# aconz2/font-ocr

Hardware: AMD Instinct MI355X
Metric: Mpixels/s scanned (95-glyph x --x-bits=2 bank) (higher is better)
Workload: dtype i8

## Files before the change

### font_ocr_amd/csrc/hip/common.h

```cpp
#pragma once

#include <hip/hip_runtime.h>

#include <algorithm>
#include <cstddef>
#include <cstdint>
#include <cstdio>
#include <mutex>
#include <string>
#include <vector>

#include "devmem.h"
#include "focr_ncc.h"

namespace focr_dec {
struct VerifyRec;
}

namespace focr {

struct VerifyMeta;

struct SizeClass {
    uint32_t n_w, n_h;
// ... 99 lines not shown
    uint32_t row_max = 0;
    uint32_t seg_shift = 0;
    void reset() { *this = SizeEstimate{}; }
    double margin() const { return std::min(0.2, std::max(0.04, 3.0 * var)); }
    uint64_t row_bound() const { return (uint64_t)row_max + row_max / 4 + 16; }
    void update(const focr_ctx *c, uint64_t n_cand, uint64_t n_hits, uint64_t largest_row);
    void adopt(uint64_t sig);
    void publish(uint64_t sig) const;
    static void forget(uint64_t sig);
};

}

constexpr uint32_t COUNTER_WORDS = 64, QUEUE_XCDS = 8, QUEUE_STRIDE = 32, MAX_SCAN_QUEUES = 128;
constexpr uint32_t TAIL_DONE_WORD = 56, ORDER_DONE_WORD = 57;
constexpr uint32_t LIVE_WORD0 = 8, LIVE_WORDS = 40;
static_assert(LIVE_WORD0 + LIVE_WORDS <= TAIL_DONE_WORD && ORDER_DONE_WORD < COUNTER_WORDS, "d_counter's named words overlap");
constexpr size_t COUNTER_BYTES = (COUNTER_WORDS + (size_t)MAX_SCAN_QUEUES * QUEUE_XCDS * QUEUE_STRIDE) * sizeof(uint32_t);

struct ResultBlock {
    uint64_t candidates;
    uint64_t hits;
    uint64_t matches;
    uint64_t lines_chars;
    uint64_t flags;
    uint64_t row_max;
    uint64_t tail_hits;
    uint64_t host_hits;
};
enum ResSlot : uint32_t { RES_CANDIDATES, RES_HITS, RES_MATCHES, RES_LINES_CHARS, RES_FLAGS, RES_ROW_MAX, RES_TAIL_HITS, RES_HOST_HITS, RES_SLOTS };
static_assert(sizeof(ResultBlock) == 64 && sizeof(ResultBlock) == RES_SLOTS * sizeof(uint64_t), "the result block is eight words");
static_assert(offsetof(ResultBlock, candidates) == 8 * RES_CANDIDATES && offsetof(ResultBlock, hits) == 8 * RES_HITS && offsetof(ResultBlock, matches) == 8 * RES_MATCHES &&
// ... 212 lines not shown
                     unsigned long long capacity, int rust);
int reserve_hits(focr_ctx *c, size_t want);
int launch_scan_mfma(focr_ctx *ctx, float threshold);
int launch_clear(focr_ctx *c, const focr::ClearList &l);
int pass_stats(focr_ctx *c, const ScanPlan &P, size_t si, double thr_d);
bool pass_appends(const focr_ctx *c, const SuperClass &su);
int build_mfma_bank(focr_ctx *ctx, const uint8_t *needles);
void layout_supers(focr_ctx *c);
int quantise_bank(focr_ctx *c, const uint8_t *dense, std::vector<int8_t> &qbank, std::vector<uint32_t> &tglobal, std::vector<uint32_t> &order_of);
bool rows_applicable(const focr_ctx *c);
uint32_t rows_capacity_for(uint64_t row_max);
void row_segments(const focr_ctx *c, uint32_t *seg_shift, uint32_t *n_seg);
size_t row_buckets(const focr_ctx *c);
unsigned tail_grid(const focr_ctx *c, unsigned blocks);
int rows2_begin(focr_ctx *c, ClearList &clear);
int rows2_place(focr_ctx *c, const unsigned long long *n_cand_p, size_t ub_c, size_t ub_h, bool big_expected, bool sort);
int rows2_verify(focr_ctx *c, double thr_d, const unsigned long long *n_cand_p, size_t ub_c);
int legacy_verify(focr_ctx *c, double thr_d, const unsigned long long *n_cand_p, size_t ub_c, float *sims, uint64_t *flags);
int sort_keys_u64(focr_ctx *c, DevArray<uint64_t> &keys, DevArray<uint64_t> &keys_alt, size_t n, unsigned end_bit);
int sort_pairs_u64_f32(focr_ctx *c, DevArray<uint64_t> &keys, DevArray<uint64_t> &keys_alt, DevArray<float> &vals, DevArray<float> &vals_alt, size_t n, unsigned end_bit);
int exclusive_scan_u64(focr_ctx *c, const uint64_t *in, uint64_t *out, size_t n);
int compact_candidates(focr_ctx *c, const uint64_t *keys, const float *sims, const uint64_t *flags, uint64_t *pos,
                       const unsigned long long *n_cand_p, size_t ub_c);
int order_sorted_hits(focr_ctx *c, uint64_t *hkeys, float *hsims, const uint64_t *n_p, size_t ub, const unsigned long long *n_cand_p, size_t ub_c);
int order_hits(focr_ctx *ctx);
int materialise_matches(focr_ctx *c, hipStream_t s);
void bank_host_prepare(focr_ctx *c, const focr_template_t *templates, size_t n_templates, const uint8_t *needles,
                       std::vector<uint32_t> &direct, std::vector<uint8_t> &dense);
void ctx_share_stream(focr_ctx *c, hipStream_t lane_stream, hipStream_t io_stream);
int wait_batch(focr_ctx *c);
int pages_alt_ingest(focr_ctx *c, const void *d_luma, size_t n_pages, size_t r_w, size_t r_h, int invert, hipStream_t s);
int pages_alt_swap(focr_ctx *c, size_t n_pages, size_t r_w, size_t r_h);
// ... 35 lines not shown
```

### font_ocr_amd/csrc/hip/ctx.hip

```cpp
#include <algorithm>
#include <cmath>
#include <cstring>
#include <mutex>

#include "common.h"

namespace focr {

static std::mutex g_err_mu;
static std::string g_err;

void set_global_error(const std::string &s) {
    std::lock_guard<std::mutex> lk(g_err_mu);
    g_err = s;
}

int fail(focr_ctx *ctx, int code, const std::string &msg) {
    if (ctx) ctx->err = msg;
    set_global_error(msg);
    return code;
}

static void free_bank(focr_ctx *c) {
    c->bank = {};
// ... 141 lines not shown

int focr_debug_set_tail_grid(focr_ctx_t *c, uint32_t num, uint32_t den) {
    if (!c) return FOCR_ERR_INVALID;
    c->dbg_grid_num = num;
    c->dbg_grid_den = den;
    return FOCR_OK;
}

int focr_debug_set_stats_form(focr_ctx_t *c, int form) {
    if (!c || form < 0 || form > 1) return FOCR_ERR_INVALID;
    c->dbg_stats_form = form;
    return FOCR_OK;
}

int focr_debug_set_verify_form(focr_ctx_t *c, int form) {
    if (!c || form < 0 || form > 1) return FOCR_ERR_INVALID;
    c->dbg_verify_form = form;
    return FOCR_OK;
}

int focr_sync(focr_ctx_t *c) {
    if (!c) return FOCR_ERR_INVALID;
    FOCR_HIP(c, hipSetDevice(c->device));
    if (c->sizes_pending || c->post_pending) return finish_results(c);
    return wait_batch(c);
}

int focr_bank_upload(focr_ctx_t *c, const focr_template_t *templates, size_t n_templates, const uint8_t *needles,
                     size_t needles_len) {
    if (!c || !templates || !n_templates || !needles) return fail(c, FOCR_ERR_INVALID, "focr_bank_upload: bad arguments");
    if (n_templates > 65535) return fail(c, FOCR_ERR_INVALID, "focr_bank_upload: more than 65535 templates");
// ... 145 lines not shown
```

### font_ocr_amd/csrc/hip/rows.hip

```cpp
#include "common.h"

namespace focr {

constexpr uint32_t XBINS = 1024;
template <int CAP, int WAVES, bool LIST, bool PAY>
__global__ __launch_bounds__(WAVES * 64) void row_sort_kernel(uint32_t n_rows, const uint32_t *__restrict__ base, const uint32_t *__restrict__ fill,
                                                              uint64_t *__restrict__ bucket, uint32_t sub_bits, uint32_t bt, uint32_t seg_mask, uint32_t xs, uint32_t n_bins,
                                                              uint32_t *__restrict__ big, unsigned long long *__restrict__ flags_word, float *__restrict__ pay,
                                                              unsigned long long limit) {
    extern __shared__ __attribute__((aligned(16))) uint32_t sort_lds[];
    constexpr int K = CAP / 64;
    const int lane = threadIdx.x & 63, wv = threadIdx.x >> 6;
    uint32_t *cur = sort_lds + (size_t)wv * (XBINS + 1 + CAP);
    uint32_t *out = cur + XBINS + 1;
    const uint32_t wave = __builtin_amdgcn_readfirstlane(blockIdx.x * WAVES + wv), n_waves = gridDim.x * WAVES;
    const uint64_t sub_mask = (1ull << sub_bits) - 1;
    const uint32_t n_items = LIST ? min(big[0], n_rows) : n_rows;
    uint32_t it = wave, r = 0, n = 0, b = 0;
    if (it < n_items) {
        r = LIST ? big[1 + it] : it;
        n = fill[r];
        b = base[r];
    }
    while (it < n_items) {
// ... 73 lines not shown
#pragma unroll
            for (int k = 0; k < K; k++)
                if (64u * k < n && (uint32_t)lane + 64u * k < n) {
                    const uint32_t e = sub[k], bin = ((e >> bt) & seg_mask) >> xs, lo = cur[bin], hi = cur[bin + 1];
                    uint32_t rank = 0;
                    for (uint32_t i = lo; i < hi; i++) rank += out[i] < e;
                    row[lo + rank] = high | e;
                    if (PAY) pay[b + lo + rank] = pv[k];
                }
            __builtin_amdgcn_fence(__ATOMIC_ACQ_REL, "wavefront");
        }
        it = it2, r = r2, n = n2, b = b2;
    }
}

__global__ __launch_bounds__(256) void hit_scatter_kernel(const uint64_t *__restrict__ cand, const unsigned long long *__restrict__ n_cand_p, unsigned long long cap,
                                                          const RowHist rows, const uint32_t *__restrict__ hbase, const float *__restrict__ sims,
                                                          const uint32_t *__restrict__ slots, uint64_t *__restrict__ hkeys, float *__restrict__ hsims,
                                                          unsigned long long hit_cap) {
    const unsigned long long n = min(*n_cand_p, cap);
    const unsigned long long stride = (unsigned long long)gridDim.x * blockDim.x;
    for (unsigned long long i = (unsigned long long)blockIdx.x * blockDim.x + threadIdx.x; i < n; i += stride) {
        const uint32_t slot = slots[i];
        if (slot == 0xffffffffu) continue;
        const uint64_t key = cand[i];
        const unsigned long long pos = (unsigned long long)hbase[row_of_key(key, rows)] + slot;
        if (pos < hit_cap) {
            hkeys[pos] = key;
            hsims[pos] = sims[i];
        }
    }
}


void row_segments(const focr_ctx *c, uint32_t *seg_shift, uint32_t *n_seg) {
    uint32_t sh = c->est.seg_shift;
    if (!sh) {
        while (((size_t)1 << sh) < c->pages.r_w) sh++;
        while (sh > 5 && ((size_t)1 << sh) * c->n_templates > ((size_t)1 << 19)) sh--;
    }
    *seg_shift = sh;
    *n_seg = (uint32_t)((c->pages.r_w + ((size_t)1 << sh) - 1) >> sh);
}

// ... 20 lines not shown
    if (!clear.add(big, 8)) return fail(c, FOCR_ERR_INVALID, "rows: clear list full or region too large");
    uint32_t seg_shift, n_seg;
    row_segments(c, &seg_shift, &n_seg);
    c->row_hist = RowHist{nullptr, (uint32_t)c->pages.r_h, c->fmt.bt + c->fmt.bx, c->fmt.by, (uint32_t)c->sub_p0, c->fmt.bt, c->fmt.bx, seg_shift, n_seg};
    return FOCR_OK;
}

uint32_t rows_capacity_for(uint64_t row_max) { return row_max <= 4096 ? 4096u : 0u; }

unsigned tail_grid(const focr_ctx *c, unsigned blocks) {
    if (!c->dbg_grid_num || !c->dbg_grid_den) return blocks;
    return (unsigned)std::max<uint64_t>(1, (uint64_t)blocks * c->dbg_grid_num / c->dbg_grid_den);
}


int rows2_place(focr_ctx *c, const unsigned long long *n_cand_p, size_t ub_c, size_t ub_h, bool big_expected, bool sort) {
    const uint32_t n_rows = (uint32_t)row_buckets(c);
    int rc;
    if ((rc = reserve_hits(c, ub_h + 1))) return rc;
    const unsigned cus = c->n_cus;
    const uint32_t *hits = (const uint32_t *)c->rows_hits.p, *hbase = (const uint32_t *)c->rows_hbase.p;
    if (ub_c) {
        const unsigned nb = tail_grid(c, (unsigned)std::max<size_t>(1, std::min<size_t>((ub_c + 255) / 256, (size_t)cus * 16)));
        hipLaunchKernelGGL(hit_scatter_kernel, dim3(nb), dim3(256), 0, c->stream, (const uint64_t *)c->d_cand, n_cand_p, (unsigned long long)ub_c, c->row_hist, hbase,
                           (const float *)c->scan_pos.p, (const uint32_t *)c->scan_flags.p, c->d_hit_keys, c->d_hit_sims_alt, (unsigned long long)c->d_hit_keys.cap);
        FOCR_HIP(c, hipGetLastError());
    }
    if (!sort) return FOCR_OK;
    unsigned long long *flags_word = (unsigned long long *)&c->d_res.p->flags;
    const unsigned row_blocks = tail_grid(c, (unsigned)std::max<size_t>(1, std::min<size_t>(((size_t)n_rows + 3) / 4, (size_t)cus * 8)));
    const uint32_t seg_w = 1u << c->row_hist.seg_shift;
    uint32_t xs = 0;
    while ((seg_w >> xs) > XBINS) xs++;
    const uint32_t n_bins = seg_w >> xs;
    uint32_t *big = (uint32_t *)c->rows_big.p;
    auto k1 = row_sort_kernel<1024, 4, false, true>;
    auto k2 = row_sort_kernel<4096, 1, true, true>;
    const size_t lds1 = (size_t)4 * (XBINS + 1 + 1024) * 4, lds2 = (size_t)(XBINS + 1 + 4096) * 4;
    hipLaunchKernelGGL(k1, dim3(row_blocks), dim3(256), lds1, c->stream, n_rows, hbase, hits, c->d_hit_keys, c->fmt.bt + c->fmt.bx, c->fmt.bt, seg_w - 1, xs, n_bins,
                       big_expected ? big : (uint32_t *)nullptr, flags_word, c->d_hit_sims_alt, (unsigned long long)c->d_hit_keys.cap);
// ... 11 lines not shown
```

### font_ocr_amd/csrc/hip/scan_mfma.hip

```cpp
#include <algorithm>
#include <cmath>
#include <mutex>

#include "mfma_common.h"

namespace focr {

struct TurnChain {
    std::mutex mu;
    static constexpr unsigned RING = 8;
    hipEvent_t ev[RING] = {};
    unsigned n = 0;
};
static TurnChain scan_turns[64], stats_turns[64];

struct Turn {
    focr_ctx *c;
    TurnChain &chain;
    std::lock_guard<std::mutex> lock;
    bool entered = false;
    Turn(focr_ctx *c, TurnChain &chain) : c(c), chain(chain), lock(chain.mu) {}
    int begin() {
        for (hipEvent_t &e : chain.ev)
            if (!e) FOCR_HIP(c, hipEventCreateWithFlags(&e, hipEventDisableTiming));
// ... 145 lines not shown
                }
                if (rc) return rc;
                t0 = t1;
            }
        }
    }
    for (size_t k = 0; k < c->bank.classes.size(); k++) {
        const SizeClass &sc = c->bank.classes[k];
        if (!sc.tall || sc.n_w >= c->pages.r_w || sc.n_h >= c->pages.r_h) continue;
        if ((rc = launch_scan_tall(c, k, thr_d, c->d_cand, nullptr, c->d_counter.as<unsigned long long>() + 1, (unsigned long long)c->ub_cand, 0))) return rc;
    }
    return FOCR_OK;
}

static int row_tail(focr_ctx *c, double thr_d, const unsigned long long *n_cand_p, size_t ub_c) {
    int rc = rows2_verify(c, thr_d, n_cand_p, ub_c);
    if (rc) return rc;
    size_t ub_h = std::min(ub_c, c->est.hits);
    uint64_t row_max = c->est.row_bound();
    if (!c->estimated) {
        uint64_t hits = 0;
        FOCR_HIP(c, hipMemcpyAsync(&hits, &c->d_res.p->tail_hits, sizeof(uint64_t), hipMemcpyDeviceToHost, c->stream));
        FOCR_HIP(c, hipMemcpyAsync(&row_max, &c->d_res.p->row_max, sizeof(uint64_t), hipMemcpyDeviceToHost, c->stream));
        FOCR_HIP(c, hipStreamSynchronize(c->stream));
        ub_h = (size_t)hits;
    }
    c->row_cap = rows_capacity_for(row_max);
    const bool big_expected = row_max > 1024, sort_rows = c->row_cap != 0;
    c->tail_path.big_launch = sort_rows && big_expected;
    c->tail_path.library_sort = !sort_rows && ub_h >= 2;
    c->tail_path.seg_shift = c->row_hist.seg_shift;
    c->tail_path.n_seg = c->row_hist.n_seg;
    if ((rc = rows2_place(c, n_cand_p, ub_c, ub_h, big_expected, sort_rows))) return rc;
    if (!sort_rows && (rc = sort_pairs_u64_f32(c, c->d_hit_keys, c->d_hit_keys_alt, c->d_hit_sims_alt, c->d_hit_sims, ub_h, c->fmt.bits()))) return rc;
    return order_sorted_hits(c, c->d_hit_keys, c->d_hit_sims_alt, &c->d_res.p->tail_hits, ub_h, n_cand_p, ub_c);
}

static int legacy_tail(focr_ctx *c, double thr_d, const unsigned long long *n_cand_p, size_t ub_c) {
    c->row_cap = 0;
    int rc = reserve_hits(c, ub_c + 1);
    if (rc) return rc;
    if (!c->scratch(c->scan_flags, (ub_c + 1) * 8) || !c->scratch(c->scan_pos, (ub_c + 1) * 8)) return fail(c, FOCR_ERR_NOMEM, "scan_mfma: hipMalloc failed");
    uint64_t *flags = c->scan_flags.as<uint64_t>(), *pos = c->scan_pos.as<uint64_t>();
    if (c->d_cand_alt.reserve(c->d_cand.cap, Grow::exact, &c->stream)) return fail(c, FOCR_ERR_NOMEM, "scan_mfma: hipMalloc(cand_alt) failed");
    if ((rc = sort_keys_u64(c, c->d_cand, c->d_cand_alt, ub_c, c->fmt.bits()))) return rc;
    if ((rc = legacy_verify(c, thr_d, n_cand_p, ub_c, c->d_hit_sims, flags))) return rc;
    FOCR_HIP(c, hipEventRecord(c->ev[EV_VERIFY_END], c->stream));
    if ((rc = compact_candidates(c, c->d_cand, c->d_hit_sims, flags, pos, n_cand_p, ub_c))) return rc;
// ... 64 lines not shown
```

### font_ocr_amd/csrc/hip/verify.h

```cpp
#pragma once
#include "common.h"

namespace focr {

typedef int v4i __attribute__((ext_vector_type(4)));
typedef v4i v4i_b1 __attribute__((aligned(1)));
typedef int v3i __attribute__((ext_vector_type(3)));
typedef v3i v3i_b1 __attribute__((aligned(1)));
typedef unsigned int v2u __attribute__((ext_vector_type(2)));

struct VerifyMeta {
    double s_n, n_recip, rnorm_n;
    uint16_t n_w, n_h;
    uint32_t row0;
};
static_assert(sizeof(VerifyMeta) == 32, "VerifyMeta is staged in LDS as two 16-byte words per template (verify_plan.h: VERIFY_RECORD_BYTES)");
struct VerifyArgs {
    const uint8_t *pages;
    uint32_t pitch, rows_alloc;
    KeyFmt fmt;
    const uint32_t *order_of;
    const TemplateConst *tc;
    const v4i *needles16;
    const uint32_t *needle16_row;
// ... 35 lines not shown
    const uint32_t r = emit ? row_of_key(key, rows) : 0xffffffffu;
    uint32_t slot = 0xffffffffu;
    uint64_t todo = __builtin_amdgcn_ballot_w64(emit);
    while (todo) {
        const uint32_t r0 = (uint32_t)__builtin_amdgcn_readlane((int)r, (int)__builtin_ctzll(todo));
        const uint64_t peers = __builtin_amdgcn_ballot_w64(r == r0);
        uint32_t start = 0;
        if (lane == (int)__builtin_ctzll(peers)) start = atomicAdd(row_hits + r0, (uint32_t)__builtin_popcountll(peers));
        start = (uint32_t)__builtin_amdgcn_readlane((int)start, (int)__builtin_ctzll(peers));
        if (r == r0) slot = start + __builtin_amdgcn_mbcnt_hi((uint32_t)(peers >> 32), __builtin_amdgcn_mbcnt_lo((uint32_t)peers, 0u));
        todo &= ~peers;
    }
    return slot;
}


__device__ __forceinline__ bool verify_candidate(uint64_t key, const VerifyArgs &va, float *sim_out) {
    const VerifyFrame f = verify_frame(key, va);
    if (f.bad) return verify_reject(va, sim_out);
    const uint32_t ci = va.order_of[f.t];
    const TemplateConst c = va.tc[ci];
    const uint32_t halves = c.n_w > 16 ? 2 : 1;
    const uint32_t row0 = va.needle16_row[ci];
    const v4i *nd = va.needles16 + row0;
    const uint8_t *pg = f.window(va);
    uint32_t acc = 0, s_p = 0, s2_p = 0;
    for (uint32_t hf = 0; hf < halves; hf++) {
        const uint32_t w_here = min(c.n_w - 16 * hf, 16u);
        v4i keep;
#pragma unroll
// ... 137 lines not shown
```

### font_ocr_amd/csrc/hip/verify.hip

```cpp
#include "tail_block.h"
#include "verify.h"
#include "verify_plan.h"

namespace focr {

static VerifyArgs verify_args(const focr_ctx *c, double thr_d) {
    return VerifyArgs{c->pages.u8, (uint32_t)c->pages.pitch, (uint32_t)c->pages.rows_alloc, c->fmt, c->bank.d_order_of, c->bank.d_tconst,
                      c->bank.d_needles16.as<const v4i>(), c->bank.d_needle16_row, thr_d, c->bank.d_vmeta.p,
                      (uint32_t)c->n_templates, (uint32_t)c->n_pages,
                      (uint32_t)c->pages.r_w, (uint32_t)c->pages.r_h, (unsigned long long *)&c->d_res.p->flags};
}

__global__ __launch_bounds__(1024) void row_prefix_kernel(const uint32_t *__restrict__ cnt, uint32_t n, uint32_t *__restrict__ base,
                                                          uint32_t *__restrict__ zero, uint64_t *__restrict__ total_out,
                                                          uint64_t *__restrict__ max_out) {
    __shared__ uint32_t wave_sum[16], wave_max[16];
    row_prefix_block(cnt, n, base, zero, total_out, max_out, wave_sum, wave_max);
}

template <int MODE>
__global__ __launch_bounds__(VERIFY_THREADS, MODE >= 2 ? 8 : 1) void verify_list_kernel(
    const uint64_t *__restrict__ cand, const unsigned long long *__restrict__ n_cand_p, unsigned long long cap, const VerifyArgs va, uint32_t lds_rows, uint32_t n_h,
    const RowHist rows, float *__restrict__ sims, uint32_t *__restrict__ slots, uint32_t *__restrict__ row_hits, const TailWork tw) {
    extern __shared__ __attribute__((aligned(16))) v4i verify_lds[];
    __shared__ uint32_t wave_sum[16], wave_max[16];
    constexpr bool LDS = MODE == 1;
    VerifyMeta *meta = reinterpret_cast<VerifyMeta *>(verify_lds);
    v4i *needle_lds = verify_lds + 2 * va.n_templates;
    uint32_t *needle12 = reinterpret_cast<uint32_t *>(needle_lds);
    v2u *needle8 = reinterpret_cast<v2u *>(needle_lds + va.n_templates);
    for (uint32_t i = threadIdx.x; i < 2 * va.n_templates; i += blockDim.x) verify_lds[i] = reinterpret_cast<const v4i *>(va.vmeta)[i];
    if (MODE == 1)
        for (uint32_t i = threadIdx.x; i < lds_rows; i += blockDim.x) needle_lds[i] = va.needles16[i];
    if (MODE == 2)
        for (uint32_t i = threadIdx.x; i < lds_rows; i += blockDim.x) {
            const v4i r = va.needles16[i];
            needle12[3 * i] = (uint32_t)r[0], needle12[3 * i + 1] = (uint32_t)r[1], needle12[3 * i + 2] = (uint32_t)r[2];
        }
// ... 5 lines not shown
        for (uint32_t i = threadIdx.x; i < 4 * va.n_templates; i += blockDim.x) {
            const uint32_t t = i >> 2, q = i & 3, row0 = va.vmeta[t].row0;
            uint32_t d = 0;
#pragma unroll
            for (uint32_t k = 0; k < 4; k++)
                if (4 * q + k < n_h) d |= ((uint32_t)va.needles16[row0 + 4 * q + k][2] & 0xffu) << (8 * k);
            reinterpret_cast<uint32_t *>(needle_lds)[i] = d;
        }
    }
    __syncthreads();
    const unsigned long long n = min(*n_cand_p, cap);
    const int lane = threadIdx.x & 63;
    const unsigned long long stride = (unsigned long long)gridDim.x * blockDim.x;
    const unsigned long long first = (unsigned long long)blockIdx.x * blockDim.x + (threadIdx.x & ~63u);
    uint64_t key_next = first + lane < n ? cand[first + lane] : 0;
    for (unsigned long long i0 = first; i0 < n; i0 += stride) {
        const unsigned long long i = i0 + lane;
        const bool valid = i < n;
        const uint64_t key = key_next;
        if (i + stride < n) key_next = cand[i + stride];
        float sim = 0.f;
        const bool emit = valid && (MODE == 3   ? verify_candidate_w89(key, va, needle8, needle_lds, meta, &sim)
                                    : MODE == 2 ? verify_candidate_narrow(key, va, needle12, meta, &sim)
                                                : verify_candidate_meta<LDS>(key, va, needle_lds, meta, &sim));
        const uint32_t slot = claim_slot(emit, key, rows, row_hits, lane);
        if (valid) {
            sims[i] = sim;
            slots[i] = slot;
        }
    }
    if (last_workgroup(tw.done)) row_prefix_block(row_hits, tw.n_rows, tw.hbase, nullptr, tw.total_out, tw.max_out, wave_sum, wave_max);
}

template <int ROWB>
__global__ __launch_bounds__(VERIFY_THREADS, 4) void verify_chunks_kernel(
    const uint64_t *__restrict__ cand, const unsigned long long *__restrict__ n_cand_p, unsigned long long cap, const VerifyArgs va, const ChunkTable ct,
    const uint32_t *__restrict__ vrows_t, const VerifyMeta *__restrict__ vmeta_t, const RowHist rows, float *__restrict__ sims, uint32_t *__restrict__ slots,
    uint32_t *__restrict__ row_hits, const TailWork tw) {
    extern __shared__ __attribute__((aligned(16))) v4i verify_lds[];
    __shared__ uint32_t wave_sum[16], wave_max[16];
    constexpr uint32_t ROWDW = ROWB / 4;
    VerifyMeta *meta = reinterpret_cast<VerifyMeta *>(verify_lds);
    const int lane = threadIdx.x & 63, wv = threadIdx.x >> 6;
    uint64_t *q_base = reinterpret_cast<uint64_t *>(verify_lds + ct.data_bytes / 16);
    uint64_t *q_key = q_base + (size_t)wv * CHUNK_QUEUE;
    uint32_t *q_pos = reinterpret_cast<uint32_t *>(q_base + (size_t)(VERIFY_THREADS / 64) * CHUNK_QUEUE) + (size_t)wv * CHUNK_QUEUE;
    const unsigned long long n = min(*n_cand_p, cap);
    const unsigned long long n_waves = (unsigned long long)gridDim.x * (VERIFY_THREADS / 64);
    const unsigned long long per_wave = ((n + n_waves - 1) / n_waves + 63) / 64 * 64;
    const unsigned long long wb = min(n, ((unsigned long long)blockIdx.x * (VERIFY_THREADS / 64) + wv) * per_wave), we = min(n, wb + per_wave);
    auto step = [&](uint32_t m, const VerifyMeta *meta_c, const uint32_t *rows_c) {
        const bool valid = (uint32_t)lane < m;
        const uint64_t key = valid ? q_key[lane] : 0;
        const uint32_t pos = valid ? q_pos[lane] : 0;
        float sim = 0.f;
        bool emit = false;
        if (valid) {
            if (ROWB == 12) emit = verify_candidate_narrow(key, va, rows_c, meta_c, &sim);
            else emit = verify_candidate_meta<true>(key, va, reinterpret_cast<const v4i *>(rows_c), meta_c, &sim);
        }
        const uint32_t slot = claim_slot(emit, key, rows, row_hits, lane);
        if (valid && pos < n) {
            sims[pos] = sim;
            slots[pos] = slot;
        }
    };
    for (uint32_t k = 0; k < ct.n; k++) {
        const uint32_t t_lo = ct.t_lo[k], t_hi = ct.t_lo[k + 1], row_lo = ct.row_lo[k], n_rows_c = ct.row_lo[k + 1] - row_lo;
        uint32_t *rows_lds = reinterpret_cast<uint32_t *>(verify_lds + 2 * (t_hi - t_lo));
        __syncthreads();
        for (uint32_t i = threadIdx.x; i < 2 * (t_hi - t_lo); i += VERIFY_THREADS) verify_lds[i] = reinterpret_cast<const v4i *>(vmeta_t + t_lo)[i];
        for (uint32_t i = threadIdx.x; i < n_rows_c * ROWDW; i += VERIFY_THREADS) rows_lds[i] = vrows_t[(size_t)row_lo * ROWDW + i];
        __syncthreads();
        const VerifyMeta *meta_c = meta - t_lo;
        const uint32_t *rows_c = rows_lds - (size_t)row_lo * ROWDW;
        uint32_t count = 0;
        for (unsigned long long i0 = wb; i0 < we; i0 += 4 * 64) {
            uint64_t key4[4];
#pragma unroll
            for (int q = 0; q < 4; q++) {
                const unsigned long long i = i0 + 64 * q + lane;
                key4[q] = i < we ? cand[i] : ~0ull;
            }
#pragma unroll
            for (int q = 0; q < 4; q++) {
                const unsigned long long i = i0 + 64 * q + lane;
                const bool valid = i < we;
                const uint64_t key = key4[q];
                const uint32_t t = va.fmt.t(key);
                const bool in = valid && ((t >= t_lo && t < t_hi) || (k + 1 == ct.n && t >= t_hi));
                const uint64_t mask = __builtin_amdgcn_ballot_w64(in);
                if (mask) {
                    if (in) {
                        const uint32_t p = count + __builtin_amdgcn_mbcnt_hi((uint32_t)(mask >> 32), __builtin_amdgcn_mbcnt_lo((uint32_t)mask, 0u));
                        q_key[p] = key;
                        q_pos[p] = (uint32_t)i;
                    }
                    count += (uint32_t)__builtin_popcountll(mask);
                    __builtin_amdgcn_fence(__ATOMIC_ACQ_REL, "wavefront");
                    if (count >= 64) {
                        step(64, meta_c, rows_c);
                        const uint32_t rest = count - 64;
                        const uint64_t kk = (uint32_t)lane < rest ? q_key[64 + lane] : 0;
                        const uint32_t pp = (uint32_t)lane < rest ? q_pos[64 + lane] : 0;
                        __builtin_amdgcn_fence(__ATOMIC_ACQ_REL, "wavefront");
                        if ((uint32_t)lane < rest) {
                            q_key[lane] = kk;
                            q_pos[lane] = pp;
                        }
                        count = rest;
                        __builtin_amdgcn_fence(__ATOMIC_ACQ_REL, "wavefront");
                    }
                }
            }
        }
        if (count) step(count, meta_c, rows_c);
        __builtin_amdgcn_fence(__ATOMIC_ACQ_REL, "wavefront");
    }
    if (last_workgroup(tw.done)) row_prefix_block(row_hits, tw.n_rows, tw.hbase, nullptr, tw.total_out, tw.max_out, wave_sum, wave_max);
}

__global__ __launch_bounds__(256) void verify_kernel(const uint64_t *__restrict__ cand, const unsigned long long *__restrict__ n_cand_p, unsigned long long ub,
                                                     const VerifyArgs va, float *__restrict__ sims, uint64_t *__restrict__ flags) {
    unsigned long long i = (unsigned long long)blockIdx.x * blockDim.x + threadIdx.x;
    if (i > ub) return;
    if (i >= min(*n_cand_p, ub)) {
        flags[i] = 0;
        return;
    }
    float sim;
    const bool emit = verify_candidate(cand[i], va, &sim);
    sims[i] = sim;
    flags[i] = emit ? 1 : 0;
}


int legacy_verify(focr_ctx *c, double thr_d, const unsigned long long *n_cand_p, size_t ub_c, float *sims, uint64_t *flags) {
    hipLaunchKernelGGL(verify_kernel, dim3((unsigned)((ub_c + 1 + 255) / 256)), dim3(256), 0, c->stream, c->d_cand, n_cand_p, (unsigned long long)ub_c,
                       verify_args(c, thr_d), sims, flags);
    FOCR_HIP(c, hipGetLastError());
    return FOCR_OK;
}

struct VerifyLaunch {
    const unsigned long long *n_cand_p;
    size_t ub_c;
    VerifyArgs va;
    float *sims;
    uint32_t *slots, *hits;
    TailWork tw;
    unsigned blocks(const focr_ctx *c, size_t most) const {
        return tail_grid(c, (unsigned)std::max<size_t>(1, std::min<size_t>((ub_c + VERIFY_THREADS - 1) / VERIFY_THREADS, most)));
    }
};

template <int ROWB>
static bool launch_chunks_rowb(focr_ctx *c, const VerifyPlan &P, const VerifyLaunch &L) {
    if (hipFuncSetAttribute(reinterpret_cast<const void *>(verify_chunks_kernel<ROWB>), hipFuncAttributeMaxDynamicSharedMemorySize, (int)P.lds) != hipSuccess) {
        (void)hipGetLastError();
        return false;
    }
    hipLaunchKernelGGL(verify_chunks_kernel<ROWB>, dim3(L.blocks(c, c->n_cus)), dim3(VERIFY_THREADS), P.lds, c->stream, (const uint64_t *)c->d_cand, L.n_cand_p,
                       (unsigned long long)L.ub_c, L.va, P.chunks, c->bank.d_vrows_t.as<const uint32_t>(), c->bank.d_vmeta_t.p, c->row_hist, L.sims, L.slots, L.hits, L.tw);
    return true;
}
static bool launch_chunks(focr_ctx *c, const VerifyPlan &P, const VerifyLaunch &L) {
    return c->bank.vrow_bytes == 12 ? launch_chunks_rowb<12>(c, P, L) : launch_chunks_rowb<16>(c, P, L);
}

template <int MODE>
static void launch_list_mode(focr_ctx *c, const VerifyPlan &P, const VerifyLaunch &L, unsigned nb) {
    (void)hipFuncSetAttribute(reinterpret_cast<const void *>(verify_list_kernel<MODE>), hipFuncAttributeMaxDynamicSharedMemorySize, (int)P.lds);
    hipLaunchKernelGGL(verify_list_kernel<MODE>, dim3(nb), dim3(VERIFY_THREADS), P.lds, c->stream, (const uint64_t *)c->d_cand, L.n_cand_p, (unsigned long long)L.ub_c, L.va,
                       P.rows, P.n_h, c->row_hist, L.sims, L.slots, L.hits, L.tw);
}
static void launch_list(focr_ctx *c, const VerifyPlan &P, const VerifyLaunch &L) {
    const unsigned cus = c->n_cus;
    const unsigned vcus = (c->scan_cus && c->scan_cus < cus && !c->tail_full_chip) ? std::max(cus - c->scan_cus, cus / 16) : cus;
    const unsigned nb = L.blocks(c, (size_t)vcus * P.per_cu);
    switch (P.form) {
        case FOCR_VERIFY_FORM_LDS8: launch_list_mode<3>(c, P, L, nb); break;
        case FOCR_VERIFY_FORM_LDS12: launch_list_mode<2>(c, P, L, nb); break;
        case FOCR_VERIFY_FORM_LDS16: launch_list_mode<1>(c, P, L, nb); break;
        default: launch_list_mode<0>(c, P, L, nb); break;
    }
}

int rows2_verify(focr_ctx *c, double thr_d, const unsigned long long *n_cand_p, size_t ub_c) {
    const uint32_t n_rows = (uint32_t)row_buckets(c);
    if (!c->scratch(c->scan_pos, (ub_c + 1) * 4) || !c->scratch(c->scan_flags, (ub_c + 1) * 4)) return fail(c, FOCR_ERR_NOMEM, "rows: hipMalloc failed");
    uint32_t *hits = c->rows_hits, *hbase = c->rows_hbase;
    if (ub_c) {
        VerifyPlan P = plan_verify(c->bank.h_tconst, c->bank.vrow_bytes, c->bank.h_vrow0_t.data(), c->dbg_verify_form);
        const VerifyLaunch L{n_cand_p, ub_c, verify_args(c, thr_d), c->scan_pos.as<float>(), c->scan_flags.as<uint32_t>(), hits,
                             TailWork{c->d_counter + TAIL_DONE_WORD, n_rows, hbase, &c->d_res.p->tail_hits, &c->d_res.p->row_max}};
        if (P.form == FOCR_VERIFY_FORM_CHUNKS && !launch_chunks(c, P, L)) P = verify_plan_global(c->n_templates);
        if (P.form != FOCR_VERIFY_FORM_CHUNKS) launch_list(c, P, L);
        FOCR_HIP(c, hipGetLastError());
        c->tail_path.verify_form = P.form;
        c->tail_path.verify_chunks = P.chunks.n;
    }
    FOCR_HIP(c, hipEventRecord(c->ev[EV_VERIFY_END], c->stream));
    if (!ub_c) {
        hipLaunchKernelGGL(row_prefix_kernel, dim3(1), dim3(1024), 0, c->stream, (const uint32_t *)hits, n_rows, hbase, (uint32_t *)nullptr, &c->d_res.p->tail_hits, &c->d_res.p->row_max);
        FOCR_HIP(c, hipGetLastError());
    }
    return FOCR_OK;
}

// ... 2 lines not shown
```

### font_ocr_amd/csrc/hip/verify_plan.h

```cpp
#pragma once
#include <algorithm>
#include <cstddef>
#include <cstdint>

#include "focr_ncc.h"

namespace focr {

constexpr unsigned VERIFY_THREADS = 1024;
constexpr uint32_t MAX_VERIFY_CHUNKS = 16, CHUNK_QUEUE = 128;
struct ChunkTable {
    uint32_t n;
    uint32_t t_lo[MAX_VERIFY_CHUNKS + 1];
    uint32_t row_lo[MAX_VERIFY_CHUNKS + 1];
    uint32_t data_bytes;
};

constexpr size_t VERIFY_RECORD_BYTES = 32;
constexpr size_t VERIFY_LDS_HALF_CU = ((size_t)80 << 10) - 256;
constexpr size_t VERIFY_LDS_WHOLE = (size_t)144 << 10;
constexpr size_t VERIFY_LDS_CHUNKS = (size_t)150 << 10;
constexpr size_t VERIFY_QUEUE_BYTES = (size_t)(VERIFY_THREADS / 64) * CHUNK_QUEUE * 12 + 64;
constexpr size_t VERIFY_GLOBAL_PAIR_RECORDS = (size_t)64 << 10;

// ... 16 lines not shown
    size_t all_rows = 0, n_templates = 0;
    uint32_t max_w = 0, min_w = ~0u, h_lo = ~0u, h_hi = 0;
    for (const auto &tc : templates) {
        n_templates++;
        all_rows += (size_t)tc.n_h * (tc.n_w > 16 ? 2u : 1u);
        max_w = std::max<uint32_t>(max_w, tc.n_w);
        min_w = std::min<uint32_t>(min_w, tc.n_w);
        h_lo = std::min<uint32_t>(h_lo, tc.n_h);
        h_hi = std::max<uint32_t>(h_hi, tc.n_h);
    }
    const size_t meta_bytes = n_templates * VERIFY_RECORD_BYTES;
    const size_t w89_bytes = meta_bytes + n_templates * 16 + all_rows * 8;
    if (min_w >= 8 && max_w == 9 && h_lo == h_hi && h_hi <= 16 && (uint64_t)max_w * h_hi * 255 * 255 <= 0xffffffffull && w89_bytes <= VERIFY_LDS_HALF_CU &&
        debug_form == 0)
        return VerifyPlan{FOCR_VERIFY_FORM_LDS8, w89_bytes, (uint32_t)all_rows, h_hi, 2, ChunkTable{}};
    if (max_w <= 12 && meta_bytes + all_rows * 12 <= VERIFY_LDS_HALF_CU)
        return VerifyPlan{FOCR_VERIFY_FORM_LDS12, meta_bytes + all_rows * 12, (uint32_t)all_rows, 0, 2, ChunkTable{}};
    if (meta_bytes + all_rows * 16 <= VERIFY_LDS_WHOLE) return VerifyPlan{FOCR_VERIFY_FORM_LDS16, meta_bytes + all_rows * 16, (uint32_t)all_rows, 0, 1, ChunkTable{}};
    if (!vrow_bytes) return verify_plan_global(n_templates);
    const size_t budget = VERIFY_LDS_CHUNKS - VERIFY_QUEUE_BYTES;
    ChunkTable ct{};
    size_t bytes = 0;
    uint32_t t0 = 0;
    for (uint32_t t = 0; t <= n_templates; t++) {
        const size_t add = t < n_templates ? VERIFY_RECORD_BYTES + (size_t)(vrow0_t[t + 1] - vrow0_t[t]) * vrow_bytes : 0;
        if (t == n_templates || bytes + add > budget) {
            if (t == t0 || ct.n == MAX_VERIFY_CHUNKS) return verify_plan_global(n_templates);
            ct.t_lo[ct.n] = t0;
            ct.row_lo[ct.n] = vrow0_t[t0];
            ct.data_bytes = std::max(ct.data_bytes, (uint32_t)((bytes + 15) & ~(size_t)15));
            ct.n++;
            t0 = t;
            bytes = 0;
        }
        bytes += add;
// ... 8 lines not shown
```

Baseline: 37040.

## Compact verified hits into per-wave record blocks instead of per-candidate arrays

Verify kernels no longer write a sim and slot for every candidate. Each wave ballots its hits and appends 16-byte {key, sim, slot} records into 256-entry blocks it claims with a global atomic cursor, then pads the unused tail of its last block with empty records. The scatter kernel walks only these records, bounded by the expected hit count plus slack, rather than all candidates. This cuts verify write traffic and scatter read traffic when hits are sparse, at the cost of atomics, padding records, and extra debug plan forms.

After: 36870. About the same (-0.5%).

```diff
diff --git a/font_ocr_amd/csrc/hip/common.h b/font_ocr_amd/csrc/hip/common.h
--- a/font_ocr_amd/csrc/hip/common.h
+++ b/font_ocr_amd/csrc/hip/common.h
@@ -137,8 +137,9 @@
 
 constexpr uint32_t COUNTER_WORDS = 64, QUEUE_XCDS = 8, QUEUE_STRIDE = 32, MAX_SCAN_QUEUES = 128;
 constexpr uint32_t TAIL_DONE_WORD = 56, ORDER_DONE_WORD = 57;
+constexpr uint32_t HIT_CURSOR_WORD = 58;
 constexpr uint32_t LIVE_WORD0 = 8, LIVE_WORDS = 40;
-static_assert(LIVE_WORD0 + LIVE_WORDS <= TAIL_DONE_WORD && ORDER_DONE_WORD < COUNTER_WORDS, "d_counter's named words overlap");
+static_assert(LIVE_WORD0 + LIVE_WORDS <= TAIL_DONE_WORD && ORDER_DONE_WORD < HIT_CURSOR_WORD && HIT_CURSOR_WORD < COUNTER_WORDS, "d_counter's named words overlap");
 constexpr size_t COUNTER_BYTES = (COUNTER_WORDS + (size_t)MAX_SCAN_QUEUES * QUEUE_XCDS * QUEUE_STRIDE) * sizeof(uint32_t);
 
 struct ResultBlock {
@@ -381,8 +382,9 @@
 size_t row_buckets(const focr_ctx *c);
 unsigned tail_grid(const focr_ctx *c, unsigned blocks);
 int rows2_begin(focr_ctx *c, ClearList &clear);
-int rows2_place(focr_ctx *c, const unsigned long long *n_cand_p, size_t ub_c, size_t ub_h, bool big_expected, bool sort);
-int rows2_verify(focr_ctx *c, double thr_d, const unsigned long long *n_cand_p, size_t ub_c);
+int rows2_place(focr_ctx *c, size_t ub_rec, size_t ub_h, bool big_expected, bool sort);
+int rows2_verify(focr_ctx *c, double thr_d, const unsigned long long *n_cand_p, size_t ub_c, size_t ub_rec);
+size_t hit_record_slack(const focr_ctx *c, size_t ub_c);
 int legacy_verify(focr_ctx *c, double thr_d, const unsigned long long *n_cand_p, size_t ub_c, float *sims, uint64_t *flags);
 int sort_keys_u64(focr_ctx *c, DevArray<uint64_t> &keys, DevArray<uint64_t> &keys_alt, size_t n, unsigned end_bit);
 int sort_pairs_u64_f32(focr_ctx *c, DevArray<uint64_t> &keys, DevArray<uint64_t> &keys_alt, DevArray<float> &vals, DevArray<float> &vals_alt, size_t n, unsigned end_bit);
diff --git a/font_ocr_amd/csrc/hip/ctx.hip b/font_ocr_amd/csrc/hip/ctx.hip
--- a/font_ocr_amd/csrc/hip/ctx.hip
+++ b/font_ocr_amd/csrc/hip/ctx.hip
@@ -179,7 +179,7 @@
 }
 
 int focr_debug_set_verify_form(focr_ctx_t *c, int form) {
-    if (!c || form < 0 || form > 1) return FOCR_ERR_INVALID;
+    if (!c || form < 0 || form > 4) return FOCR_ERR_INVALID;
     c->dbg_verify_form = form;
     return FOCR_OK;
 }
diff --git a/font_ocr_amd/csrc/hip/rows.hip b/font_ocr_amd/csrc/hip/rows.hip
--- a/font_ocr_amd/csrc/hip/rows.hip
+++ b/font_ocr_amd/csrc/hip/rows.hip
@@ -1,4 +1,5 @@
 #include "common.h"
+#include "verify.h"
 
 namespace focr {
 
@@ -111,20 +112,18 @@
     }
 }
 
-__global__ __launch_bounds__(256) void hit_scatter_kernel(const uint64_t *__restrict__ cand, const unsigned long long *__restrict__ n_cand_p, unsigned long long cap,
-                                                          const RowHist rows, const uint32_t *__restrict__ hbase, const float *__restrict__ sims,
-                                                          const uint32_t *__restrict__ slots, uint64_t *__restrict__ hkeys, float *__restrict__ hsims,
-                                                          unsigned long long hit_cap) {
-    const unsigned long long n = min(*n_cand_p, cap);
+__global__ __launch_bounds__(256) void hit_scatter_kernel(const HitRecord *__restrict__ recs, const uint32_t *__restrict__ n_rec_p, unsigned long long rec_cap,
+                                                          const RowHist rows, const uint32_t *__restrict__ hbase, uint64_t *__restrict__ hkeys,
+                                                          float *__restrict__ hsims, unsigned long long hit_cap) {
+    const unsigned long long n = min((unsigned long long)*n_rec_p, rec_cap);
     const unsigned long long stride = (unsigned long long)gridDim.x * blockDim.x;
     for (unsigned long long i = (unsigned long long)blockIdx.x * blockDim.x + threadIdx.x; i < n; i += stride) {
-        const uint32_t slot = slots[i];
-        if (slot == 0xffffffffu) continue;
-        const uint64_t key = cand[i];
-        const unsigned long long pos = (unsigned long long)hbase[row_of_key(key, rows)] + slot;
+        const HitRecord r = recs[i];
+        if (r.slot == HIT_EMPTY) continue;
+        const unsigned long long pos = (unsigned long long)hbase[row_of_key(r.key, rows)] + r.slot;
         if (pos < hit_cap) {
-            hkeys[pos] = key;
-            hsims[pos] = sims[i];
+            hkeys[pos] = r.key;
+            hsims[pos] = r.sim;
         }
     }
 }
@@ -175,16 +174,17 @@
 }
 
 
-int rows2_place(focr_ctx *c, const unsigned long long *n_cand_p, size_t ub_c, size_t ub_h, bool big_expected, bool sort) {
+int rows2_place(focr_ctx *c, size_t ub_rec, size_t ub_h, bool big_expected, bool sort) {
     const uint32_t n_rows = (uint32_t)row_buckets(c);
     int rc;
     if ((rc = reserve_hits(c, ub_h + 1))) return rc;
     const unsigned cus = c->n_cus;
     const uint32_t *hits = (const uint32_t *)c->rows_hits.p, *hbase = (const uint32_t *)c->rows_hbase.p;
-    if (ub_c) {
-        const unsigned nb = tail_grid(c, (unsigned)std::max<size_t>(1, std::min<size_t>((ub_c + 255) / 256, (size_t)cus * 16)));
-        hipLaunchKernelGGL(hit_scatter_kernel, dim3(nb), dim3(256), 0, c->stream, (const uint64_t *)c->d_cand, n_cand_p, (unsigned long long)ub_c, c->row_hist, hbase,
-                           (const float *)c->scan_pos.p, (const uint32_t *)c->scan_flags.p, c->d_hit_keys, c->d_hit_sims_alt, (unsigned long long)c->d_hit_keys.cap);
+    const size_t n_walk = ub_h ? std::min(ub_rec, ub_h + hit_record_slack(c, c->ub_cand)) : 0;
+    if (n_walk) {
+        const unsigned nb = tail_grid(c, (unsigned)std::max<size_t>(1, std::min<size_t>((n_walk + 255) / 256, (size_t)cus * 16)));
+        hipLaunchKernelGGL(hit_scatter_kernel, dim3(nb), dim3(256), 0, c->stream, (const HitRecord *)c->scan_pos.as<HitRecord>(), (const uint32_t *)(c->d_counter + HIT_CURSOR_WORD),
+                           (unsigned long long)ub_rec, c->row_hist, hbase, c->d_hit_keys, c->d_hit_sims_alt, (unsigned long long)c->d_hit_keys.cap);
         FOCR_HIP(c, hipGetLastError());
     }
     if (!sort) return FOCR_OK;
diff --git a/font_ocr_amd/csrc/hip/scan_mfma.hip b/font_ocr_amd/csrc/hip/scan_mfma.hip
--- a/font_ocr_amd/csrc/hip/scan_mfma.hip
+++ b/font_ocr_amd/csrc/hip/scan_mfma.hip
@@ -183,9 +183,10 @@
 }
 
 static int row_tail(focr_ctx *c, double thr_d, const unsigned long long *n_cand_p, size_t ub_c) {
-    int rc = rows2_verify(c, thr_d, n_cand_p, ub_c);
+    size_t ub_h = std::min(ub_c, c->est.hits);
+    const size_t ub_rec = (c->estimated ? ub_h + 1 : ub_c) + hit_record_slack(c, ub_c);
+    int rc = rows2_verify(c, thr_d, n_cand_p, ub_c, ub_rec);
     if (rc) return rc;
-    size_t ub_h = std::min(ub_c, c->est.hits);
     uint64_t row_max = c->est.row_bound();
     if (!c->estimated) {
         uint64_t hits = 0;
@@ -200,7 +201,7 @@
     c->tail_path.library_sort = !sort_rows && ub_h >= 2;
     c->tail_path.seg_shift = c->row_hist.seg_shift;
     c->tail_path.n_seg = c->row_hist.n_seg;
-    if ((rc = rows2_place(c, n_cand_p, ub_c, ub_h, big_expected, sort_rows))) return rc;
+    if ((rc = rows2_place(c, ub_rec, ub_h, big_expected, sort_rows))) return rc;
     if (!sort_rows && (rc = sort_pairs_u64_f32(c, c->d_hit_keys, c->d_hit_keys_alt, c->d_hit_sims_alt, c->d_hit_sims, ub_h, c->fmt.bits()))) return rc;
     return order_sorted_hits(c, c->d_hit_keys, c->d_hit_sims_alt, &c->d_res.p->tail_hits, ub_h, n_cand_p, ub_c);
 }
diff --git a/font_ocr_amd/csrc/hip/verify.h b/font_ocr_amd/csrc/hip/verify.h
--- a/font_ocr_amd/csrc/hip/verify.h
+++ b/font_ocr_amd/csrc/hip/verify.h
@@ -73,6 +73,43 @@
     return slot;
 }
 
+constexpr uint32_t HIT_BLOCK = 256, HIT_EMPTY = 0xffffffffu;
+struct HitRecord {
+    uint64_t key;
+    float sim;
+    uint32_t slot;
+};
+static_assert(sizeof(HitRecord) == 16, "a hit record is one 16-byte store");
+struct HitList {
+    HitRecord *recs;
+    uint32_t *cursor;
+    unsigned long long cap;
+};
+struct HitBlock {
+    uint32_t base = 0, used = HIT_BLOCK;
+};
+__device__ __forceinline__ void emit_hit_records(bool emit, uint64_t key, float sim, uint32_t slot, const HitList &hl, HitBlock &hb, int lane) {
+    const uint64_t hits = __builtin_amdgcn_ballot_w64(emit);
+    if (!hits) return;
+    const uint32_t cnt = (uint32_t)__builtin_popcountll(hits), rest = HIT_BLOCK - hb.used;
+    const uint32_t rank = __builtin_amdgcn_mbcnt_hi((uint32_t)(hits >> 32), __builtin_amdgcn_mbcnt_lo((uint32_t)hits, 0u));
+    uint32_t next = 0;
+    if (cnt > rest) {
+        if (lane == 0) next = atomicAdd(hl.cursor, HIT_BLOCK);
+        next = (uint32_t)__builtin_amdgcn_readfirstlane((int)next);
+    }
+    const unsigned long long pos = rank < rest ? (unsigned long long)hb.base + hb.used + rank : (unsigned long long)next + (rank - rest);
+    if (emit && pos < hl.cap) hl.recs[pos] = HitRecord{key, sim, slot};
+    if (cnt > rest) hb.base = next, hb.used = cnt - rest;
+    else hb.used += cnt;
+}
+__device__ __forceinline__ void close_hit_records(const HitList &hl, const HitBlock &hb, int lane) {
+    for (uint32_t i = hb.used + (uint32_t)lane; i < HIT_BLOCK; i += 64) {
+        const unsigned long long pos = (unsigned long long)hb.base + i;
+        if (pos < hl.cap) hl.recs[pos] = HitRecord{0, 0.f, HIT_EMPTY};
+    }
+}
+
 
 __device__ __forceinline__ bool verify_candidate(uint64_t key, const VerifyArgs &va, float *sim_out) {
     const VerifyFrame f = verify_frame(key, va);
diff --git a/font_ocr_amd/csrc/hip/verify.hip b/font_ocr_amd/csrc/hip/verify.hip
--- a/font_ocr_amd/csrc/hip/verify.hip
+++ b/font_ocr_amd/csrc/hip/verify.hip
@@ -21,7 +21,7 @@
 template <int MODE>
 __global__ __launch_bounds__(VERIFY_THREADS, MODE >= 2 ? 8 : 1) void verify_list_kernel(
     const uint64_t *__restrict__ cand, const unsigned long long *__restrict__ n_cand_p, unsigned long long cap, const VerifyArgs va, uint32_t lds_rows, uint32_t n_h,
-    const RowHist rows, float *__restrict__ sims, uint32_t *__restrict__ slots, uint32_t *__restrict__ row_hits, const TailWork tw) {
+    const RowHist rows, const HitList hl, uint32_t *__restrict__ row_hits, const TailWork tw) {
     extern __shared__ __attribute__((aligned(16))) v4i verify_lds[];
     __shared__ uint32_t wave_sum[16], wave_max[16];
     constexpr bool LDS = MODE == 1;
@@ -57,6 +57,7 @@
     const unsigned long long stride = (unsigned long long)gridDim.x * blockDim.x;
     const unsigned long long first = (unsigned long long)blockIdx.x * blockDim.x + (threadIdx.x & ~63u);
     uint64_t key_next = first + lane < n ? cand[first + lane] : 0;
+    HitBlock hb;
     for (unsigned long long i0 = first; i0 < n; i0 += stride) {
         const unsigned long long i = i0 + lane;
         const bool valid = i < n;
@@ -66,20 +67,17 @@
         const bool emit = valid && (MODE == 3   ? verify_candidate_w89(key, va, needle8, needle_lds, meta, &sim)
                                     : MODE == 2 ? verify_candidate_narrow(key, va, needle12, meta, &sim)
                                                 : verify_candidate_meta<LDS>(key, va, needle_lds, meta, &sim));
-        const uint32_t slot = claim_slot(emit, key, rows, row_hits, lane);
-        if (valid) {
-            sims[i] = sim;
-            slots[i] = slot;
-        }
-    }
+        emit_hit_records(emit, key, sim, claim_slot(emit, key, rows, row_hits, lane), hl, hb, lane);
+    }
+    close_hit_records(hl, hb, lane);
     if (last_workgroup(tw.done)) row_prefix_block(row_hits, tw.n_rows, tw.hbase, nullptr, tw.total_out, tw.max_out, wave_sum, wave_max);
 }
 
 template <int ROWB>
 __global__ __launch_bounds__(VERIFY_THREADS, 4) void verify_chunks_kernel(
     const uint64_t *__restrict__ cand, const unsigned long long *__restrict__ n_cand_p, unsigned long long cap, const VerifyArgs va, const ChunkTable ct,
-    const uint32_t *__restrict__ vrows_t, const VerifyMeta *__restrict__ vmeta_t, const RowHist rows, float *__restrict__ sims, uint32_t *__restrict__ slots,
-    uint32_t *__restrict__ row_hits, const TailWork tw) {
+    const uint32_t *__restrict__ vrows_t, const VerifyMeta *__restrict__ vmeta_t, const RowHist rows, const HitList hl, uint32_t *__restrict__ row_hits,
+    const TailWork tw) {
     extern __shared__ __attribute__((aligned(16))) v4i verify_lds[];
     __shared__ uint32_t wave_sum[16], wave_max[16];
     constexpr uint32_t ROWDW = ROWB / 4;
@@ -87,26 +85,21 @@
     const int lane = threadIdx.x & 63, wv = threadIdx.x >> 6;
     uint64_t *q_base = reinterpret_cast<uint64_t *>(verify_lds + ct.data_bytes / 16);
     uint64_t *q_key = q_base + (size_t)wv * CHUNK_QUEUE;
-    uint32_t *q_pos = reinterpret_cast<uint32_t *>(q_base + (size_t)(VERIFY_THREADS / 64) * CHUNK_QUEUE) + (size_t)wv * CHUNK_QUEUE;
     const unsigned long long n = min(*n_cand_p, cap);
     const unsigned long long n_waves = (unsigned long long)gridDim.x * (VERIFY_THREADS / 64);
     const unsigned long long per_wave = ((n + n_waves - 1) / n_waves + 63) / 64 * 64;
     const unsigned long long wb = min(n, ((unsigned long long)blockIdx.x * (VERIFY_THREADS / 64) + wv) * per_wave), we = min(n, wb + per_wave);
+    HitBlock hb;
     auto step = [&](uint32_t m, const VerifyMeta *meta_c, const uint32_t *rows_c) {
         const bool valid = (uint32_t)lane < m;
         const uint64_t key = valid ? q_key[lane] : 0;
-        const uint32_t pos = valid ? q_pos[lane] : 0;
         float sim = 0.f;
         bool emit = false;
         if (valid) {
             if (ROWB == 12) emit = verify_candidate_narrow(key, va, rows_c, meta_c, &sim);
             else emit = verify_candidate_meta<true>(key, va, reinterpret_cast<const v4i *>(rows_c), meta_c, &sim);
         }
-        const uint32_t slot = claim_slot(emit, key, rows, row_hits, lane);
-        if (valid && pos < n) {
-            sims[pos] = sim;
-            slots[pos] = slot;
-        }
+        emit_hit_records(emit, key, sim, claim_slot(emit, key, rows, row_hits, lane), hl, hb, lane);
     };
     for (uint32_t k = 0; k < ct.n; k++) {
         const uint32_t t_lo = ct.t_lo[k], t_hi = ct.t_lo[k + 1], row_lo = ct.row_lo[k], n_rows_c = ct.row_lo[k + 1] - row_lo;
@@ -137,7 +130,6 @@
                     if (in) {
                         const uint32_t p = count + __builtin_amdgcn_mbcnt_hi((uint32_t)(mask >> 32), __builtin_amdgcn_mbcnt_lo((uint32_t)mask, 0u));
                         q_key[p] = key;
-                        q_pos[p] = (uint32_t)i;
                     }
                     count += (uint32_t)__builtin_popcountll(mask);
                     __builtin_amdgcn_fence(__ATOMIC_ACQ_REL, "wavefront");
@@ -145,12 +137,8 @@
                         step(64, meta_c, rows_c);
                         const uint32_t rest = count - 64;
                         const uint64_t kk = (uint32_t)lane < rest ? q_key[64 + lane] : 0;
-                        const uint32_t pp = (uint32_t)lane < rest ? q_pos[64 + lane] : 0;
                         __builtin_amdgcn_fence(__ATOMIC_ACQ_REL, "wavefront");
-                        if ((uint32_t)lane < rest) {
-                            q_key[lane] = kk;
-                            q_pos[lane] = pp;
-                        }
+                        if ((uint32_t)lane < rest) q_key[lane] = kk;
                         count = rest;
                         __builtin_amdgcn_fence(__ATOMIC_ACQ_REL, "wavefront");
                     }
@@ -160,6 +148,7 @@
         if (count) step(count, meta_c, rows_c);
         __builtin_amdgcn_fence(__ATOMIC_ACQ_REL, "wavefront");
     }
+    close_hit_records(hl, hb, lane);
     if (last_workgroup(tw.done)) row_prefix_block(row_hits, tw.n_rows, tw.hbase, nullptr, tw.total_out, tw.max_out, wave_sum, wave_max);
 }
 
@@ -189,8 +178,8 @@
     const unsigned long long *n_cand_p;
     size_t ub_c;
     VerifyArgs va;
-    float *sims;
-    uint32_t *slots, *hits;
+    HitList hl;
+    uint32_t *hits;
     TailWork tw;
     unsigned blocks(const focr_ctx *c, size_t most) const {
         return tail_grid(c, (unsigned)std::max<size_t>(1, std::min<size_t>((ub_c + VERIFY_THREADS - 1) / VERIFY_THREADS, most)));
@@ -204,7 +193,7 @@
         return false;
     }
     hipLaunchKernelGGL(verify_chunks_kernel<ROWB>, dim3(L.blocks(c, c->n_cus)), dim3(VERIFY_THREADS), P.lds, c->stream, (const uint64_t *)c->d_cand, L.n_cand_p,
-                       (unsigned long long)L.ub_c, L.va, P.chunks, c->bank.d_vrows_t.as<const uint32_t>(), c->bank.d_vmeta_t.p, c->row_hist, L.sims, L.slots, L.hits, L.tw);
+                       (unsigned long long)L.ub_c, L.va, P.chunks, c->bank.d_vrows_t.as<const uint32_t>(), c->bank.d_vmeta_t.p, c->row_hist, L.hl, L.hits, L.tw);
     return true;
 }
 static bool launch_chunks(focr_ctx *c, const VerifyPlan &P, const VerifyLaunch &L) {
@@ -215,7 +204,7 @@
 static void launch_list_mode(focr_ctx *c, const VerifyPlan &P, const VerifyLaunch &L, unsigned nb) {
     (void)hipFuncSetAttribute(reinterpret_cast<const void *>(verify_list_kernel<MODE>), hipFuncAttributeMaxDynamicSharedMemorySize, (int)P.lds);
     hipLaunchKernelGGL(verify_list_kernel<MODE>, dim3(nb), dim3(VERIFY_THREADS), P.lds, c->stream, (const uint64_t *)c->d_cand, L.n_cand_p, (unsigned long long)L.ub_c, L.va,
-                       P.rows, P.n_h, c->row_hist, L.sims, L.slots, L.hits, L.tw);
+                       P.rows, P.n_h, c->row_hist, L.hl, L.hits, L.tw);
 }
 static void launch_list(focr_ctx *c, const VerifyPlan &P, const VerifyLaunch &L) {
     const unsigned cus = c->n_cus;
@@ -229,13 +218,18 @@
     }
 }
 
-int rows2_verify(focr_ctx *c, double thr_d, const unsigned long long *n_cand_p, size_t ub_c) {
+size_t hit_record_slack(const focr_ctx *c, size_t ub_c) {
+    const size_t waves = (size_t)tail_grid(c, std::max(1u, 2 * c->n_cus)) * (VERIFY_THREADS / 64);
+    return std::min(waves, ub_c / 64 + 1) * HIT_BLOCK;
+}
+
+int rows2_verify(focr_ctx *c, double thr_d, const unsigned long long *n_cand_p, size_t ub_c, size_t ub_rec) {
     const uint32_t n_rows = (uint32_t)row_buckets(c);
-    if (!c->scratch(c->scan_pos, (ub_c + 1) * 4) || !c->scratch(c->scan_flags, (ub_c + 1) * 4)) return fail(c, FOCR_ERR_NOMEM, "rows: hipMalloc failed");
+    if (!c->scratch(c->scan_pos, (ub_rec + 1) * sizeof(HitRecord))) return fail(c, FOCR_ERR_NOMEM, "rows: hipMalloc failed");
     uint32_t *hits = c->rows_hits, *hbase = c->rows_hbase;
     if (ub_c) {
         VerifyPlan P = plan_verify(c->bank.h_tconst, c->bank.vrow_bytes, c->bank.h_vrow0_t.data(), c->dbg_verify_form);
-        const VerifyLaunch L{n_cand_p, ub_c, verify_args(c, thr_d), c->scan_pos.as<float>(), c->scan_flags.as<uint32_t>(), hits,
+        const VerifyLaunch L{n_cand_p, ub_c, verify_args(c, thr_d), HitList{c->scan_pos.as<HitRecord>(), c->d_counter + HIT_CURSOR_WORD, (unsigned long long)ub_rec}, hits,
                              TailWork{c->d_counter + TAIL_DONE_WORD, n_rows, hbase, &c->d_res.p->tail_hits, &c->d_res.p->row_max}};
         if (P.form == FOCR_VERIFY_FORM_CHUNKS && !launch_chunks(c, P, L)) P = verify_plan_global(c->n_templates);
         if (P.form != FOCR_VERIFY_FORM_CHUNKS) launch_list(c, P, L);
diff --git a/font_ocr_amd/csrc/hip/verify_plan.h b/font_ocr_amd/csrc/hip/verify_plan.h
--- a/font_ocr_amd/csrc/hip/verify_plan.h
+++ b/font_ocr_amd/csrc/hip/verify_plan.h
@@ -54,11 +54,17 @@
     if (min_w >= 8 && max_w == 9 && h_lo == h_hi && h_hi <= 16 && (uint64_t)max_w * h_hi * 255 * 255 <= 0xffffffffull && w89_bytes <= VERIFY_LDS_HALF_CU &&
         debug_form == 0)
         return VerifyPlan{FOCR_VERIFY_FORM_LDS8, w89_bytes, (uint32_t)all_rows, h_hi, 2, ChunkTable{}};
-    if (max_w <= 12 && meta_bytes + all_rows * 12 <= VERIFY_LDS_HALF_CU)
+    if (debug_form == 3) return verify_plan_global(n_templates);
+    if (debug_form < 2 && max_w <= 12 && meta_bytes + all_rows * 12 <= VERIFY_LDS_HALF_CU)
         return VerifyPlan{FOCR_VERIFY_FORM_LDS12, meta_bytes + all_rows * 12, (uint32_t)all_rows, 0, 2, ChunkTable{}};
-    if (meta_bytes + all_rows * 16 <= VERIFY_LDS_WHOLE) return VerifyPlan{FOCR_VERIFY_FORM_LDS16, meta_bytes + all_rows * 16, (uint32_t)all_rows, 0, 1, ChunkTable{}};
+    if (debug_form != 4 && meta_bytes + all_rows * 16 <= VERIFY_LDS_WHOLE)
+        return VerifyPlan{FOCR_VERIFY_FORM_LDS16, meta_bytes + all_rows * 16, (uint32_t)all_rows, 0, 1, ChunkTable{}};
     if (!vrow_bytes) return verify_plan_global(n_templates);
-    const size_t budget = VERIFY_LDS_CHUNKS - VERIFY_QUEUE_BYTES;
+    size_t budget = VERIFY_LDS_CHUNKS - VERIFY_QUEUE_BYTES;
+    if (debug_form == 4) {
+        const size_t one = VERIFY_RECORD_BYTES + (size_t)2 * h_hi * vrow_bytes;
+        budget = std::min(budget, (meta_bytes + (size_t)vrow0_t[n_templates] * vrow_bytes) / 2 + one);
+    }
     ChunkTable ct{};
     size_t bytes = 0;
     uint32_t t0 = 0;
```
